# mailgun/gubernator

Hardware: AMD Instinct MI355X
Metric: rate-limit decisions/sec (kernel path, inputs resident in HBM) (higher is better)
Workload: dtype int64

## Files before the change

gubernator_amd/csrc/guber_engine.hip:

```cpp
#include <hip/hip_runtime.h>

#include <algorithm>
#include <atomic>
#include <chrono>
#include <cstdio>
#include <cstdlib>
#include <cstring>
#include <memory>
#include <mutex>
#include <string>
#include <thread>
#include <unordered_map>
#include <vector>

#include "../../include/guber_gpu.h"
#include "guber_host.h"
#include "guber_test_flags.h"
#include "guber_kernels.h"
#include "guber_kernels_lru.h"
#include "guber_item_conv.h"
#include <hipcub/hipcub.hpp>

using namespace guber;

// ... 119 lines not shown
    DevBuf<LruCtl> lru_ctl; PinBuf<LruCtl> lru_hctl;
    DevBuf<unsigned long long> lru_tstamp, lru_tstamp_in, lru_cnt; DevBuf<uint32_t> lru_tslot, lru_tslot_in; DevBuf<uint8_t> lru_sort_tmp;
    DevBuf<unsigned long long> lru_u64; DevBuf<uint32_t> lru_u32; DevBuf<uint8_t> lru_u8;
    bool lru_tail_ok = false;
    uint64_t lru_admits = 0, lru_applied = 0, lru_rebuilds = 0, lru_cuts = 0, lru_passes = 0; uint32_t lru_split_at = 0;
    uint64_t touch = 0;
    static constexpr uint32_t kRb = 32;
    struct RbSlot { uint32_t seq = 0; uint64_t mark = 0; bool armed = false; };
    RbSlot rb[kRb + 1]; int rb_ride = -1;
    uint64_t added_total = 0;
    uint64_t settle_waits = 0;
    uint64_t compactions = 0;
    std::mutex mu;
    bool profiling = false;
    struct Span { int kernel; hipEvent_t a, b; hipStream_t st; };
    std::vector<Span> spans;
    std::vector<hipEvent_t> event_pool;
    double prof_ms[32] = {0}; uint64_t prof_n[32] = {0}, prof_units[32] = {0};
    std::vector<float> group_us;

    hipEvent_t get_event() {
        if (!event_pool.empty()) { hipEvent_t ev = event_pool.back(); event_pool.pop_back(); return ev; }
        hipEvent_t ev = nullptr; (void)hipEventCreate(&ev); return ev;
    }
    void span_begin(int k, uint64_t units = 0, hipStream_t st = nullptr) { if (profiling) { Span s{k, get_event(), get_event(), st ? st : stream}; (void)hipEventRecord(s.a, s.st); spans.push_back(s); prof_units[k] += units; } }
    void span_end() { if (profiling) (void)hipEventRecord(spans.back().b, spans.back().st); }

    mutable struct PendingEval* held = nullptr;
    int set_device() const { if (held) ep_flush_held(this); return hipSetDevice(device) == hipSuccess ? 0 : -1; }
};

enum { KT_FRONT = 0, KT_EVAL2, KT_RESOLVE, KT_HIST, KT_SCATTER0, KT_SCATTER, KT_HEADS, KT_EVAL, KT_FRONT_MULTI, KT_EVAL2_MULTI,
       KT_PART, KT_OWN, KT_EVAL3, KT_PART_MULTI, KT_OWN_MULTI, KT_EVAL3_MULTI, KT_EVALPART_MULTI, KT_FR_COUNT, KT_FR_SCAN, KT_FR_SCATTER, KT_FR_OUT,
       KT_FR_ELECT, KT_FR_MISSING, KT_FR_ASK, KT_FR_OUT_STORE, KT_COUNT };
static_assert(KT_COUNT <= 32, "guber_engine::prof_* hold 32 kernels");
static const char* const kKernelNames[KT_COUNT] = {"k_front", "k_eval2", "k_resolve", "k_hist", "k_scatter(first)",
                                                   "k_scatter", "k_heads", "k_eval", "k_front_multi", "k_eval2_multi",
                                                   "k_part", "k_own", "k_eval3", "k_part_multi", "k_own_multi", "k_eval3_multi", "k_evalpart_multi",
                                                   "k_fr_count", "k_fr_scan", "k_fr_scatter", "k_fr_out",
                                                   "k_fr_elect", "k_fr_missing", "k_fr_ask", "k_fr_out_store"};

static uint64_t take_stamps(guber_engine* e, uint64_t n) {
    const uint64_t b = e->seq_next;
    e->seq_next += n ? n : 1;
    e->touch = b;
    return b;
}
static uint64_t next_pow2(uint64_t v) { uint64_t p = 1; while (p < v) p <<= 1; return p; }

static void quiesce_all(guber_engine* e) { (void)hipStreamSynchronize(e->stream); }

static void note_enqueued(guber_engine* e, uint64_t n) { e->size_upper += n; e->tags_upper += n; e->added_total += n; }
static bool rb_slot_done(const guber_engine* e, uint32_t i) {
    return __atomic_load_n((volatile uint32_t*)&e->h_rb_seq.p[i], __ATOMIC_ACQUIRE) == e->rb[i].seq;
}
static bool rb_any_armed(const guber_engine* e) { for (uint32_t i = 0; i < guber_engine::kRb; ++i) if (e->rb[i].armed) return true; return false; }
static bool rb_any_launched(const guber_engine* e) {
    for (uint32_t i = 0; i < guber_engine::kRb; ++i) if (e->rb[i].armed && (int)i != e->rb_ride) return true;
    return false;
}
static void rb_disarm_all(guber_engine* e) { for (auto& s : e->rb) s.armed = false; e->rb_ride = -1; }
static void rb_fold_slot(guber_engine* e, uint32_t i) {
    DevCounters c = e->h_ctr.p[i];
    const BlockCounters* hb = e->h_bctr.p + (size_t)i * e->n_bctr;
    for (uint32_t b = 0; b < e->n_bctr; ++b) { c.over += hb[b].over; c.hits += hb[b].hits; c.misses += hb[b].misses; c.size += hb[b].size_delta; }
    const uint64_t since = e->added_total - e->rb[i].mark;
    e->last_ctr = c;
    e->tags_upper = c.tags_used + since;
    e->size_upper = (uint64_t)std::max<long long>(c.size, 0) + since;
}
static bool rb_fold_newest(guber_engine* e) {
    int best = -1;
    for (uint32_t i = 0; i < guber_engine::kRb; ++i) {
// ... 244 lines not shown
```

gubernator_amd/csrc/guber_front.h:

```cpp
#pragma once
#include "guber_kernels_wire.h"

constexpr uint32_t FRONT_ONE_PAIR_MAX = 49152;
struct guber_front {
    std::mutex mu;
    int device = 0;
    std::vector<guber_engine*> eng;
    std::vector<hipStream_t> streams;
    std::vector<int> stream_of;
    const guber::WireEnc* enc_hook = nullptr;
    hipStream_t rs = nullptr, rs2 = nullptr, os = nullptr, last_os = nullptr; int n_own_streams = 1; bool out_on_eval = false; uint32_t out_delay = 0, one_pair_max = FRONT_ONE_PAIR_MAX; bool rs_borrowed = false;
    uint32_t cap = 0, depth = 0, max_key = 0;
    uint32_t seq = 0;
    DevBuf<uint16_t> rt_table, rt_exs; DevBuf<uint64_t> rt_exh; RouteRule rule{}; bool have_rule = false;
    struct Slot {
        DevBuf<uint8_t> mem; CohBuf<FrontHost> host;
        FrIn in{};
        uint8_t *o_status = nullptr, *o_err = nullptr; int64_t *o_limit = nullptr, *o_remaining = nullptr, *o_reset = nullptr;
        hipEvent_t ev_in = nullptr, ev_out = nullptr, ev_a = nullptr; bool out_recorded = false;
        std::vector<std::unique_ptr<EvalHook>> hooks;
        CohBuf<uint8_t> h_margs; DevBuf<uint8_t> d_margs;
        uint32_t seq = 0, n = 0;
        int64_t gen = -1;
        bool dispatched = false;
    };
    std::vector<Slot> slots;
    uint64_t generations = 0, forced_flushes = 0, host_waits = 0; double host_wait_ms = 0;
    bool pre_routed = false;
    struct GenSpan { hipEvent_t a, b; };
    std::vector<GenSpan> gen_spans;
    struct StoreSide {
        uint32_t cap = 0, cells = 0;
        DevBuf<unsigned long long> tag; DevBuf<uint32_t> first, cell, tile_cnt, index; DevBuf<uint8_t> ask, engine, flags, oflags; DevBuf<Rec> after, oafter;
        DevBuf<FrStoreCtl> ctl; DevBuf<FrStoreTabs> tabs; FrStoreTabs h_tabs{}; FrStoreCtl h_ctl{};
        std::vector<hipEvent_t> ev;
        bool probed = false, active = false;
        uint32_t n = 0, cut_at = 0; const void *key_bytes = nullptr, *key_off = nullptr; int64_t now_ms = 0;
        uint64_t probes = 0, collisions = 0, cuts = 0, asked = 0, evals = 0;
    } st;
};

static size_t front_col(size_t bytes) { return (bytes + 63) & ~(size_t)63; }
struct FrontGen { guber_batch_t b; uint32_t key_stride = 0; const uint32_t* key_len = nullptr; };

extern "C" void guber_front_destroy(guber_front_t* f) {
    if (!f) return;
    (void)hipSetDevice(f->device);
    for (hipStream_t st : {f->rs, f->rs2, f->os}) if (st) (void)hipStreamSynchronize(st);
    for (auto st : f->streams) (void)hipStreamSynchronize(st);
    for (auto& s : f->slots) {
// ... 32 lines not shown
    f->have_rule = true;
    return 0;
}

extern "C" int guber_front_create(guber_engine_t* const* engines, uint32_t n_engines, const guber_route_rule_t* rule, uint32_t max_n,
                                  uint32_t depth, guber_front_t** out) {
    if (!engines || !out || !n_engines || n_engines > (uint32_t)MULTI_MEM_MAX) return fail(GUBER_E_INVALID_ARG, "1 .. 16 engines per front");
    if (n_engines > 1 && !rule) return fail(GUBER_E_INVALID_ARG, "a front over several engines needs the placement's rule");
    if (max_n == 0 || max_n > FR_MAX_N) return fail(GUBER_E_BATCH_TOO_LARGE, "a generation holds at most 4 194 304 requests");
    if (depth == 0) depth = 4;
    if (depth < 3 || depth > 16) return fail(GUBER_E_INVALID_ARG, "3 .. 16 generations in flight");
    std::unique_ptr<guber_front, void (*)(guber_front*)> f(new guber_front(), [](guber_front* p) { guber_front_destroy(p); });
    for (uint32_t j = 0; j < n_engines; ++j) {
        guber_engine* e = engines[j];
        if (!e) return fail(GUBER_E_INVALID_ARG, "null engine");
        if (e->device != engines[0]->device) return fail(GUBER_E_INVALID_ARG, "the engines of a front live on one device");
        for (uint32_t q = 0; q < j; ++q) if (engines[q] == e) return fail(GUBER_E_INVALID_ARG, "an engine twice in one front");
        f->eng.push_back(e);
        int si = -1;
        for (size_t q = 0; q < f->streams.size(); ++q) if (f->streams[q] == e->stream) si = (int)q;
        if (si < 0) { si = (int)f->streams.size(); f->streams.push_back(e->stream); }
        f->stream_of.push_back(si);
        f->max_key = j == 0 ? e->max_key : std::min(f->max_key, e->max_key);
    }
    f->device = engines[0]->device; f->cap = max_n; f->depth = depth;
    if (hipSetDevice(f->device) != hipSuccess) return fail(GUBER_E_HIP, "hipSetDevice");
    HIPCHK(hipStreamCreateWithFlags(&f->rs, hipStreamNonBlocking));
    f->n_own_streams = 1;
    if (const char* v = guber_lab_env("GUBER_FRONT_STREAMS")) f->n_own_streams = std::max(1, std::min(3, atoi(v)));
    f->out_on_eval = true;
    if (const char* v = guber_lab_env("GUBER_FRONT_OUT_ON_EVAL")) f->out_on_eval = atoi(v) != 0;
    if (const char* v = guber_lab_env("GUBER_FRONT_OUT_DELAY")) f->out_delay = (uint32_t)std::max(0, std::min(2, atoi(v)));
    if (const char* v = guber_lab_env("GUBER_FRONT_ONE_PAIR_MAX")) f->one_pair_max = (uint32_t)strtoul(v, nullptr, 10);
    f->rs2 = f->os = f->rs;
    if (f->n_own_streams >= 2) HIPCHK(hipStreamCreateWithFlags(&f->os, hipStreamNonBlocking));
    if (f->n_own_streams >= 3) HIPCHK(hipStreamCreateWithFlags(&f->rs2, hipStreamNonBlocking));
    if (rule) { const int rc = front_set_rule(f.get(), rule); if (rc) return rc; }
    else f->rule = RouteRule{1, 1, 0, 0, -1, 0, 0, 0, nullptr, nullptr, nullptr};
    const size_t cap = max_n, tiles = (cap + FR_TILE - 1) / FR_TILE;
    f->slots.resize(depth);
    for (auto& s : f->slots) {
        const size_t bytes = 3 * front_col(cap * 4 + 4) + 5 * front_col(cap * 8) + front_col(cap * 4) + 2 * front_col(cap) +
                             3 * front_col(cap * 8) + 2 * front_col(cap) +
                             front_col(cap * FR_KEY_COPY_MAX + 64) +
                             front_col(cap * 2) + 2 * front_col(tiles * MULTI_MEM_MAX * 4) + front_col(sizeof(FrontCtl));
        if (s.mem.ensure(bytes) || s.host.ensure(1)) return GUBER_E_NOMEM;
        if (f->streams.size() == 1 && n_engines > 1 && (s.h_margs.ensure(sizeof(MultiArgsMem)) || s.d_margs.ensure(sizeof(MultiArgsMem)))) return GUBER_E_NOMEM;
        uint8_t* p = s.mem.p;
        FrIn& A = s.in;
        A.d_key_off = (uint32_t*)p; p += front_col(cap * 4 + 4); A.d_key_len = (uint32_t*)p; p += front_col(cap * 4 + 4); A.d_fwd = (uint32_t*)p; p += front_col(cap * 4 + 4);
        A.d_hits = (int64_t*)p; p += front_col(cap * 8); A.d_limit = (int64_t*)p; p += front_col(cap * 8); A.d_duration = (int64_t*)p; p += front_col(cap * 8);
        A.d_burst = (int64_t*)p; p += front_col(cap * 8); A.d_created_at = (int64_t*)p; p += front_col(cap * 8);
        A.d_behavior = (uint32_t*)p; p += front_col(cap * 4); A.d_algorithm = p; p += front_col(cap); A.d_is_owner = p; p += front_col(cap);
        s.o_limit = (int64_t*)p; p += front_col(cap * 8); s.o_remaining = (int64_t*)p; p += front_col(cap * 8); s.o_reset = (int64_t*)p; p += front_col(cap * 8);
        s.o_status = p; p += front_col(cap); s.o_err = p; p += front_col(cap);
        A.d_keys = p; p += front_col(cap * FR_KEY_COPY_MAX + 64);
        A.er = (uint16_t*)p; p += front_col(cap * 2);
        A.tile_cnt = (uint32_t*)p; p += front_col(tiles * MULTI_MEM_MAX * 4); A.tile_base = (uint32_t*)p; p += front_col(tiles * MULTI_MEM_MAX * 4);
        A.ctl = (FrontCtl*)p; p += front_col(sizeof(FrontCtl));
        A.host = s.host.p;
        memset((void*)s.host.p, 0, sizeof(FrontHost));
        HIPCHK(hipMemsetAsync(A.ctl, 0, sizeof(FrontCtl), f->rs));
        HIPCHK(hipMemsetAsync(A.d_keys, 0, front_col(cap * FR_KEY_COPY_MAX + 64), f->rs));
        HIPCHK(hipEventCreateWithFlags(&s.ev_in, hipEventDisableTiming));
        HIPCHK(hipEventCreateWithFlags(&s.ev_out, hipEventDisableTiming));
        for (size_t q = 0; q < f->streams.size(); ++q) {
            s.hooks.emplace_back(new EvalHook());
            HIPCHK(hipEventCreateWithFlags(&s.hooks.back()->ev, hipEventDisableTiming));
            s.hooks.back()->st = f->streams[q];
        }
    }
    HIPCHK(hipStreamSynchronize(f->rs));
    *out = f.release();
    return GUBER_OK;
}

static int front_route_on(guber_front* f, hipStream_t st) {
    std::lock_guard<std::mutex> lk(f->mu);
    if (f->generations || f->pre_routed || f->n_own_streams != 1) return fail(GUBER_E_INVALID_ARG, "guber_front: the routing stream is chosen before the first generation");
    if (hipSetDevice(f->device) != hipSuccess) return fail(GUBER_E_HIP, "hipSetDevice");
    HIPCHK(hipStreamSynchronize(f->rs));
    HIPCHK(hipStreamDestroy(f->rs));
    f->rs = f->rs2 = f->os = st; f->rs_borrowed = true;
    return 0;
}

extern "C" int guber_front_set_rule(guber_front_t* f, const guber_route_rule_t* rule) {
    if (!f || !rule) return fail(GUBER_E_INVALID_ARG, "null argument");
    std::lock_guard<std::mutex> lk(f->mu);
    if (hipSetDevice(f->device) != hipSuccess) return fail(GUBER_E_HIP, "hipSetDevice");
    return front_set_rule(f, rule);
}

static int front_route(guber_front* f, guber_front::Slot& s, const FrontGen* fg, int64_t gen) {
    const guber_batch_t* b = &fg->b;
    hipStream_t rs = (gen & 1) ? f->rs2 : f->rs;
    if (s.out_recorded) { HIPCHK(hipStreamWaitEvent(rs, s.ev_out, 0)); s.out_recorded = false; }
    s.gen = gen; s.n = b->n; s.dispatched = false;
    s.seq = ++f->seq ? f->seq : ++f->seq;
    for (auto& h : s.hooks) { h->outstanding.store(1); h->recorded.store(false); }
    if (b->n == 0) return 0;
    FrIn& A = s.in;
    A.n = b->n; A.n_engines = (uint32_t)f->eng.size(); A.max_key = f->max_key; A.seq = s.seq;
    A.key_bytes = b->key_bytes; A.key_off = b->key_off; A.key_stride = fg->key_stride; A.key_len = fg->key_len; A.hits = b->hits; A.limit = b->limit; A.duration = b->duration;
    A.burst = b->burst; A.created_at = b->created_at; A.behavior = b->behavior; A.algorithm = b->algorithm; A.is_owner = b->is_owner;
    A.R = f->rule;
    const uint32_t tiles = (b->n + FR_TILE - 1u) / FR_TILE;
    guber_engine* e0 = f->eng[0];
    std::unique_lock<std::mutex> pl(e0->mu, std::defer_lock);
    if (e0->profiling || s.ev_a) pl.lock();
    if (s.ev_a) e0->event_pool.push_back(s.ev_a);
    s.ev_a = nullptr;
    if (e0->profiling) { s.ev_a = e0->get_event(); (void)hipEventRecord(s.ev_a, rs); }
    e0->span_begin(KT_FR_COUNT, b->n, rs);
    hipLaunchKernelGGL(k_fr_count, dim3(tiles), dim3(FR_TILE), 0, rs, A);
    e0->span_end();
    e0->span_begin(KT_FR_SCAN, b->n, rs);
    hipLaunchKernelGGL(k_fr_scan, dim3(MULTI_MEM_MAX / 4), dim3(FR_SCAN_T), 0, rs, A, tiles, (tiles + FR_SCAN_T - 1) / FR_SCAN_T);
    e0->span_end();
    e0->span_begin(KT_FR_SCATTER, b->n, rs);
    hipLaunchKernelGGL(k_fr_scatter, dim3(tiles), dim3(256), 0, rs, A);
    e0->span_end();
    if (hipGetLastError() != hipSuccess) return fail(GUBER_E_HIP, "kernel launch");
    HIPCHK(hipEventRecord(s.ev_in, rs));
    return 0;
}

static int front_out(guber_front* f, guber_front::Slot& s, guber_result_t* r) {
    if (s.n == 0) return 0;
    hipStream_t os = f->out_on_eval ? f->streams[(size_t)s.gen % f->streams.size()] : f->os;
    f->last_os = os;
    for (auto& h : s.hooks) if (h->st != os) HIPCHK(hipStreamWaitEvent(os, h->ev, 0));
    FrOut O{};
    O.n = s.n; O.er = s.in.er; O.tile_cnt = s.in.tile_cnt; O.tile_base = s.in.tile_base; O.ctl = s.in.ctl;
    O.d_status = s.o_status; O.d_err = s.o_err; O.d_limit = s.o_limit; O.d_remaining = s.o_remaining; O.d_reset_time = s.o_reset;
    O.status = r->status; O.err = r->err; O.limit = r->limit; O.remaining = r->remaining; O.reset_time = r->reset_time;
    guber_engine* e0 = f->eng[0];
    std::unique_lock<std::mutex> pl(e0->mu, std::defer_lock);
    if (e0->profiling) pl.lock();
    e0->span_begin(f->st.active ? KT_FR_OUT_STORE : KT_FR_OUT, s.n, os);
    if (f->st.active) {
        FrOutStore S{O, f->st.flags.p, f->st.after.p, f->st.oflags.p, f->st.oafter.p};
        hipLaunchKernelGGL(k_fr_out_store, dim3((s.n + FR_TILE - 1u) / FR_TILE), dim3(256), 0, os, S);
    } else if (f->enc_hook) {
        guber::WireEnc E = *f->enc_hook;
        E.fwd = s.in.d_fwd; E.d_status = O.d_status; E.d_err = O.d_err; E.d_limit = O.d_limit; E.d_remaining = O.d_remaining; E.d_reset = O.d_reset_time;
        hipLaunchKernelGGL(guber::k_wire_enc, dim3(E.nrpc), dim3(guber::WE_T), 0, os, E);
    } else
    hipLaunchKernelGGL(k_fr_out, dim3((s.n + FR_TILE - 1u) / FR_TILE), dim3(256), 0, os, O);
    e0->span_end();
    if (s.ev_a) { hipEvent_t evb = e0->get_event(); (void)hipEventRecord(evb, os); f->gen_spans.push_back({s.ev_a, evb}); s.ev_a = nullptr; }
    if (hipGetLastError() != hipSuccess) return fail(GUBER_E_HIP, "kernel launch");
    if (os != f->rs) { HIPCHK(hipEventRecord(s.ev_out, os)); s.out_recorded = true; }
    return 0;
}

static bool front_evals_launched(const guber_front::Slot& s) {
    for (auto& h : s.hooks) if (!h->recorded.load(std::memory_order_acquire)) return false;
    return true;
}

static int front_eval(guber_front* f, const FrontGen* gens, guber_result_t* results, uint32_t count, uint32_t* done, hipEvent_t after = nullptr);
extern "C" int guber_front_eval_dev(guber_front_t* f, const guber_batch_t* gens, guber_result_t* results, uint32_t count, uint32_t* done) {
    if (done) *done = 0;
    if (!f || (count && (!gens || !results))) return fail(GUBER_E_INVALID_ARG, "null argument");
    std::vector<FrontGen> g(count);
    for (uint32_t k = 0; k < count; ++k) {
        const int rc = check_batch_args(&gens[k], &results[k]);
        if (rc) return rc;
        g[k].b = gens[k];
    }
    return front_eval(f, g.data(), results, count, done);
}
static int front_eval_locked(guber_front* f, const FrontGen* gens, guber_result_t* results, uint32_t count, uint32_t* done, hipEvent_t after);
static int front_eval(guber_front* f, const FrontGen* gens, guber_result_t* results, uint32_t count, uint32_t* done, hipEvent_t after) {
    if (done) *done = 0;
    for (uint32_t k = 0; k < count; ++k) {
        if (gens[k].b.n > f->cap) return fail(GUBER_E_BATCH_TOO_LARGE, "generation larger than the front was created for");
        if (gens[k].b.greg_expire || gens[k].b.greg_duration) return fail(GUBER_E_INVALID_ARG, "a front takes its calendar intervals from the device");
// ... 8 lines not shown
    if (f->st.probed && !f->st.active) { f->st.probed = false; f->pre_routed = false; }
    const uint32_t ne = (uint32_t)f->eng.size(), D = f->depth, ahead = D - 2;
    PendSet pendset;
    bool any_ep = false;
    for (auto* e : f->eng) any_ep = any_ep || e->fuse_ep;
    PendSet* const ps = any_ep ? &pendset : nullptr;
    struct Dispatching { bool on; Dispatching(bool o) : on(o) { if (on) ++tl_ep_dispatcher; } ~Dispatching() { if (on) --tl_ep_dispatcher; } } dispatching(any_ep);
    uint32_t next_route = 0, next_out = 0, enq = 0;
    int rc = 0;
    uint64_t fp[4] = {0, 0, 0, 0};
    struct FpSpan { uint64_t* a; uint64_t t0; explicit FpSpan(uint64_t* x) : a(x), t0(dp_now()) {} ~FpSpan() { if (g_dprof) *a += dp_now() - t0; } };
    const uint64_t g0 = f->generations;
    auto slot_of = [&](uint32_t k) -> guber_front::Slot& { return f->slots[(g0 + k) % D]; };
    auto drain_outs = [&](uint32_t upto, bool force) -> int {
        while (next_out < upto) {
            guber_front::Slot& s = slot_of(next_out);
            if (!s.dispatched) break;
            if (s.n && !front_evals_launched(s)) {
                if (!force) break;
                f->forced_flushes++;
                const int r2 = pendset.flush_all();
                if (r2) return r2;
                if (!front_evals_launched(s)) return fail(GUBER_E_HIP, "guber_front: an evaluation was not launched");
            }
            const int r3 = front_out(f, s, &results[next_out]);
            if (r3) return r3;
            ++next_out;
            if (done) *done = next_out;
        }
        return 0;
    };
    std::vector<std::vector<GroupItem>> fifo(ne);
    std::vector<EvalHook*> hook_of(ne, nullptr);
    for (uint32_t k = 0; k < count && !rc; ++k) {
        while (next_route < count && next_route <= k + ahead && !rc) {
            if (next_route >= D) { rc = drain_outs(next_route - D + 1, true); if (rc) break; }
            if (next_route == 0 && f->pre_routed) f->pre_routed = false;
            else { FpSpan sp(&fp[0]); rc = front_route(f, slot_of(next_route), &gens[next_route], (int64_t)f->generations + next_route); }
            ++next_route;
        }
        if (rc) break;
        guber_front::Slot& s = slot_of(k);
        const guber_batch_t* b = &gens[k].b;
        if (s.n) {
            auto reported = [&]() {
                for (int q = 0; q <= MULTI_MEM_MAX; ++q)
                    if ((uint32_t)(__atomic_load_n((volatile unsigned long long*)&s.host.p->w[q], __ATOMIC_ACQUIRE) >> 32) != s.seq) return false;
                return true;
            };
            if (!reported()) {
                FpSpan sp(&fp[1]);
                const auto t0 = std::chrono::steady_clock::now();
                f->host_waits++;
                uint32_t spins = 0;
                while (!reported()) {
                    if (++spins > 2000) {
                        std::this_thread::yield();
                        if ((spins & 0x3ffu) == 0 && hipStreamQuery((s.gen & 1) ? f->rs2 : f->rs) != hipErrorNotReady && !reported()) {
                            rc = fail(GUBER_E_HIP, "guber_front: the routing of a generation did not report"); break;
                        }
                    }
                }
                f->host_wait_ms += std::chrono::duration<double, std::milli>(std::chrono::steady_clock::now() - t0).count();
                if (rc) break;
            }
            uint32_t counts[MULTI_MEM_MAX];
            for (int q = 0; q < MULTI_MEM_MAX; ++q) counts[q] = (uint32_t)s.host.p->w[q];
            const bool packed = !((uint32_t)s.host.p->w[MULTI_MEM_MAX] >> 8 & 1u);
            for (auto st : f->streams) { if (hipStreamWaitEvent(st, s.ev_in, 0) != hipSuccess) { rc = fail(GUBER_E_HIP, "hipStreamWaitEvent"); break; } }
            if (rc) break;
            uint32_t base = 0, total = 0;
            for (uint32_t j = 0; j < ne; ++j) {
                fifo[j].clear();
// ... 6 lines not shown
                uint32_t piece = np > 1 ? ((nj + np - 1) / np + 255u) & ~255u : cap_e;
                if (piece > cap_e) piece = cap_e;
                for (uint32_t pos = 0; pos < nj; pos += piece) {
                    const uint32_t len = std::min(piece, nj - pos), d0 = base + pos;
                    const FrIn& A = s.in;
                    BatchView B{len, 0, packed ? A.d_keys : b->key_bytes, A.d_key_off + d0, A.d_hits + d0, A.d_limit + d0, A.d_duration + d0,
                                b->burst ? A.d_burst + d0 : nullptr, b->created_at ? A.d_created_at + d0 : nullptr,
                                A.d_algorithm + d0, A.d_behavior + d0, b->is_owner ? A.d_is_owner + d0 : nullptr, nullptr, nullptr, b->now_ms,
                                0, packed ? nullptr : A.d_key_len + d0};
                    fifo[j].push_back(GroupItem{B, ResultView{s.o_status + d0, s.o_limit + d0, s.o_remaining + d0, s.o_reset + d0, s.o_err + d0},
                                                f->st.active ? f->st.flags.p + d0 : nullptr, f->st.active ? f->st.after.p + d0 : nullptr});
                }
                base += nj;
            }
            if (total != s.n) { rc = fail(GUBER_E_HIP, "guber_front: the shares do not add up to the generation"); break; }
            bool one_pair = f->streams.size() == 1 && ne > 1 && s.h_margs.p && s.n <= f->one_pair_max;
            guber_engine* og[MULTI_MEM_MAX]; GroupItem oi[MULTI_MEM_MAX]; int on = 0;
            for (uint32_t j = 0; j < ne && one_pair; ++j) {
                if (fifo[j].empty()) continue;
                one_pair = fifo[j].size() == 1 && can_fuse(f->eng[j], fifo[j][0].B.n);
                og[on] = f->eng[j]; oi[on] = fifo[j][0]; ++on;
            }
            if (one_pair && on > 1) {
                FpSpan sp(&fp[2]);
                rc = pendset.flush_all();
                int r1 = rc ? rc : launch_group_mem(og, oi, on, &enq, (MultiArgsMem*)s.h_margs.p, (MultiArgsMem*)s.d_margs.p);
                if (r1 == 1) r1 = dispatch_rounds(f->eng.data(), ne, fifo, ps, &enq, hook_of.data());
                rc = r1;
            } else { FpSpan sp(&fp[2]); rc = dispatch_rounds(f->eng.data(), ne, fifo, ps, &enq, hook_of.data()); }
        }
        s.dispatched = true;
        for (auto& h : s.hooks) h->launched();
        if (rc) break;
        { FpSpan sp(&fp[3]); rc = drain_outs(k + 1 > f->out_delay ? k + 1 - f->out_delay : 0, false); }
    }
    {
        for (uint32_t k = 0; k < next_route; ++k) {
            guber_front::Slot& s = slot_of(k);
            if (k >= next_out && !s.dispatched) { s.dispatched = true; s.n = 0; for (auto& h : s.hooks) h->launched(); }
        }
        const int rcf = pendset.flush_all();
        if (!rc) rc = rcf;
        const int rco = drain_outs(next_route, true);
        if (!rc) rc = rco;
    }
    f->generations += next_out;
    if (after && !rc && hipEventRecord(after, f->last_os ? f->last_os : f->rs) != hipSuccess) rc = fail(GUBER_E_HIP, "hipEventRecord");
    if (g_dprof && next_out) {
        fprintf(stderr, "[front] %u generations; per generation: routing enqueue %.2f us, waiting for the shares' sizes %.2f, dispatch %.2f, answers %.2f\n", next_out,
                fp[0] / 1e3 / next_out, fp[1] / 1e3 / next_out, fp[2] / 1e3 / next_out, fp[3] / 1e3 / next_out);
        if (tl_dp[6]) fprintf(stderr, "[front dispatch] %llu batches in %llu groups; per batch: wait-for-progress %.2f us, locks %.2f, preludes+plans %.2f, argument blocks %.2f, launches %.2f\n",
                (unsigned long long)tl_dp[6], (unsigned long long)tl_dp[5], tl_dp[0] / 1e3 / tl_dp[6], tl_dp[1] / 1e3 / tl_dp[6], tl_dp[2] / 1e3 / tl_dp[6],
                tl_dp[3] / 1e3 / tl_dp[6], tl_dp[4] / 1e3 / tl_dp[6]);
        for (auto& v : tl_dp) v = 0;
    }
    return rc;
}

static int front_route_ahead(guber_front* f, const FrontGen* g) {
    if (g->b.n > f->cap) return fail(GUBER_E_BATCH_TOO_LARGE, "generation larger than the front was created for");
    if (g->key_stride & 7u) return fail(GUBER_E_INVALID_ARG, "key rows are a multiple of 8 bytes apart");
    std::lock_guard<std::mutex> lk(f->mu);
    if (f->st.probed) { f->st.probed = false; f->pre_routed = false; }
    if (f->pre_routed) return fail(GUBER_E_INVALID_ARG, "guber_front: a generation is routed ahead already");
    if (hipSetDevice(f->device) != hipSuccess) return fail(GUBER_E_HIP, "hipSetDevice");
    const int rc = front_route(f, f->slots[f->generations % f->depth], g, (int64_t)f->generations);
    if (!rc) f->pre_routed = true;
    return rc;
}
// ... 243 lines not shown
```

gubernator_amd/csrc/guber_kernels_front.h:

```cpp
#pragma once

namespace guber {

constexpr uint32_t FR_PER = 4;
constexpr uint32_t FR_TILE = 256 * FR_PER;
constexpr uint32_t FR_RANK_BITS = 10;
static_assert((1u << FR_RANK_BITS) >= FR_TILE && (MULTI_MEM_MAX << FR_RANK_BITS) <= 65536, "engine and rank share sixteen bits");
constexpr uint32_t FR_SCAN_T = 1024;
constexpr uint32_t FR_SCAN_PER = 4;
constexpr uint32_t FR_MAX_N = FR_SCAN_T * FR_SCAN_PER * FR_TILE;
constexpr uint32_t FR_KEY_COPY_MAX = 32;

struct FrontCtl {
    uint32_t tot[MULTI_MEM_MAX];
    uint32_t ragged_seq;
    uint32_t pad_[15];
};
struct FrontHost { unsigned long long w[MULTI_MEM_MAX + 1]; unsigned long long pad_[15]; };
static_assert(sizeof(FrontHost) == 256, "four lines of pinned memory per slot");

struct FrIn {
    uint32_t n, n_engines, max_key, seq;
    const uint8_t* key_bytes; const uint32_t* key_off;
    uint32_t key_stride; const uint32_t* key_len;
// ... 78 lines not shown
        const uint32_t ragged = __hip_atomic_load(&A.ctl->ragged_seq, __ATOMIC_RELAXED, __HIP_MEMORY_SCOPE_AGENT) == A.seq ? 1u : 0u;
        const uint32_t len0 = fr_len0(A);
        __hip_atomic_store(&A.host->w[MULTI_MEM_MAX], (unsigned long long)A.seq << 32 | ragged << 8 | (len0 < 255u ? len0 : 255u), __ATOMIC_RELAXED, __HIP_MEMORY_SCOPE_SYSTEM);
    }
}

struct FrTile { uint32_t lbase[MULTI_MEM_MAX + 1], dofs[MULTI_MEM_MAX]; };
__device__ __forceinline__ void fr_tile_bases(FrTile& T, const FrontCtl* ctl, const uint32_t* tile_cnt, const uint32_t* tile_base, uint32_t tile) {
    const uint32_t e = threadIdx.x;
    if (e < MULTI_MEM_MAX) {
        const uint32_t* cnt = tile_cnt + (size_t)tile * MULTI_MEM_MAX;
        uint32_t s = 0, l = 0;
        for (uint32_t k = 0; k < e; ++k) { s += ctl->tot[k]; l += cnt[k]; }
        T.lbase[e] = l; T.dofs[e] = s + tile_base[(size_t)tile * MULTI_MEM_MAX + e] - l;
        if (e == MULTI_MEM_MAX - 1) T.lbase[MULTI_MEM_MAX] = l + cnt[e];
    }
    __syncthreads();
}
__device__ __forceinline__ uint32_t fr_engine_of(const FrTile& T, uint32_t j) {
    uint32_t e = 0;
#pragma unroll
    for (uint32_t q = 1; q < MULTI_MEM_MAX; ++q) e += T.lbase[q] <= j ? 1u : 0u;
    return e;
}
__device__ __forceinline__ void fr_sorted_places(const FrTile& T, uint32_t n, uint32_t (&dd)[FR_PER]) {
    const uint32_t cnt = T.lbase[MULTI_MEM_MAX] < FR_TILE ? T.lbase[MULTI_MEM_MAX] : FR_TILE;
#pragma unroll
    for (int k = 0; k < FR_PER; ++k) {
        const uint32_t j = threadIdx.x + k * 256u, d = T.dofs[fr_engine_of(T, j)] + j;
        dd[k] = j < cnt && d < n ? d : 0xffffffffu;
    }
}

__global__ __launch_bounds__(256) void k_fr_scatter(FrIn A) {
    __shared__ FrTile T;
    __shared__ uint64_t stg[2][FR_TILE];
    const uint32_t tile = blockIdx.x, tid = threadIdx.x, i0 = tile * FR_TILE + tid;
    fr_tile_bases(T, A.ctl, A.tile_cnt, A.tile_base, tile);
    const bool packed = A.ctl->ragged_seq != A.seq;
    const uint32_t len0 = fr_len0(A), ko0 = A.key_stride ? 0u : A.key_off[0], kstep = A.key_stride ? A.key_stride : len0;
    uint32_t p[FR_PER], o0[FR_PER], klen[FR_PER]; uint64_t hits[FR_PER], limit[FR_PER], duration[FR_PER], misc[FR_PER], kw[FR_PER];
    auto word_at = [](uint32_t w, uint32_t len) { return 8u * w + 8u <= len || len < 8u ? 8u * w : len - 8u; };
#pragma unroll
    for (int k = 0; k < FR_PER; ++k) {
        const uint32_t i = i0 + k * 256u;
        p[k] = 0xffffffffu; o0[k] = klen[k] = 0; hits[k] = limit[k] = duration[k] = misc[k] = kw[k] = 0;
        if (i >= A.n) continue;
        const uint32_t er = A.er[i];
        if (packed) { o0[k] = ko0 + i * kstep; klen[k] = len0; kw[k] = ld_key_word(A.key_bytes + o0[k]); }
        else { o0[k] = fr_key_off(A, i); klen[k] = fr_key_len(A, i, o0[k]); }
        hits[k] = (uint64_t)A.hits[i]; limit[k] = (uint64_t)A.limit[i]; duration[k] = (uint64_t)A.duration[i];
        misc[k] = (A.behavior ? A.behavior[i] : 0u) | (uint64_t)(A.algorithm ? A.algorithm[i] : (uint8_t)0) << 32 | (uint64_t)(A.is_owner ? A.is_owner[i] : (uint8_t)0) << 40;
        const uint32_t e = er >> FR_RANK_BITS;
        p[k] = T.lbase[e] + (er & ((1u << FR_RANK_BITS) - 1u));
        const uint32_t d = T.dofs[e] + p[k];
        A.d_fwd[i] = d < A.n ? d : 0u;
    }
    uint32_t dd[FR_PER];
    fr_sorted_places(T, A.n, dd);
    uint32_t turn = 0;
    auto through = [&](const uint64_t (&v)[FR_PER], uint64_t (&o)[FR_PER]) {
        uint64_t* buf = stg[turn++ & 1u];
#pragma unroll
        for (int k = 0; k < FR_PER; ++k) if (p[k] < FR_TILE) buf[p[k]] = v[k];
        __syncthreads();
#pragma unroll
        for (int k = 0; k < FR_PER; ++k) o[k] = dd[k] != 0xffffffffu ? buf[threadIdx.x + k * 256u] : 0ull;
    };
    auto column = [&](const uint64_t (&v)[FR_PER], int64_t* dst) {
        uint64_t o[FR_PER];
        through(v, o);
#pragma unroll
        for (int k = 0; k < FR_PER; ++k) if (dd[k] != 0xffffffffu) dst[dd[k]] = (int64_t)o[k];
    };
    uint64_t opt[FR_PER] = {0, 0, 0, 0}, o[FR_PER];
    auto request = [&](const int64_t* src) {
#pragma unroll
        for (int k = 0; k < FR_PER; ++k) if (p[k] != 0xffffffffu) opt[k] = (uint64_t)src[i0 + k * 256u];
    };
    column(hits, A.d_hits);
    column(limit, A.d_limit);
    if (A.burst) request(A.burst);
    column(duration, A.d_duration);
    if (A.burst) column(opt, A.d_burst);
    if (A.created_at) request(A.created_at);
    through(misc, o);
#pragma unroll
    for (int k = 0; k < FR_PER; ++k) {
        if (dd[k] == 0xffffffffu) continue;
// ... 4 lines not shown
    if (packed) {
        const uint32_t nw = (len0 + 7u) >> 3;
        for (uint32_t w = 0; w < nw; ++w) {
            uint64_t next[FR_PER] = {0, 0, 0, 0};
            if (w + 1 < nw) {
#pragma unroll
                for (int k = 0; k < FR_PER; ++k) if (p[k] != 0xffffffffu) next[k] = ld_key_word(A.key_bytes + o0[k] + word_at(w + 1, len0));
            }
            through(kw, o);
#pragma unroll
            for (int k = 0; k < FR_PER; ++k) {
                kw[k] = next[k];
                if (dd[k] == 0xffffffffu) continue;
                uint8_t* dst = A.d_keys + (size_t)dd[k] * len0;
                if (len0 >= 8) __builtin_memcpy(dst + word_at(w, len0), &o[k], 8);
                else for (uint32_t q = 0; q < len0; ++q) dst[q] = (uint8_t)(o[k] >> (8 * q));
            }
        }
#pragma unroll
        for (int k = 0; k < FR_PER; ++k) {
            if (dd[k] == 0xffffffffu) continue;
            A.d_key_off[dd[k]] = dd[k] * len0;
            if (dd[k] == A.n - 1) A.d_key_off[A.n] = A.n * len0;
        }
    } else {
        uint64_t ol[FR_PER];
#pragma unroll
        for (int k = 0; k < FR_PER; ++k) ol[k] = o0[k] | (uint64_t)klen[k] << 32;
        through(ol, o);
#pragma unroll
        for (int k = 0; k < FR_PER; ++k) if (dd[k] != 0xffffffffu) { A.d_key_off[dd[k]] = (uint32_t)o[k]; A.d_key_len[dd[k]] = (uint32_t)(o[k] >> 32); }
    }
}

struct FrOut {
    uint32_t n; const uint16_t* er; const uint32_t *tile_cnt, *tile_base; const FrontCtl* ctl;
    const uint8_t *d_status, *d_err; const int64_t *d_limit, *d_remaining, *d_reset_time;
    uint8_t *status, *err; int64_t *limit, *remaining, *reset_time;
};
__global__ __launch_bounds__(256) void k_fr_out(FrOut A) {
    __shared__ FrTile T;
    __shared__ uint64_t stg[2][FR_TILE];
    __shared__ uint16_t sse[FR_TILE];
    const uint32_t tile = blockIdx.x, tid = threadIdx.x, i0 = tile * FR_TILE + tid;
    fr_tile_bases(T, A.ctl, A.tile_cnt, A.tile_base, tile);
    uint32_t dd[FR_PER], p[FR_PER]; uint16_t se[FR_PER]; int64_t l[FR_PER], r[FR_PER], t[FR_PER];
    fr_sorted_places(T, A.n, dd);
#pragma unroll
    for (int k = 0; k < FR_PER; ++k) {
        p[k] = 0xffffffffu;
        if (i0 + k * 256u < A.n) { const uint32_t er = A.er[i0 + k * 256u]; p[k] = T.lbase[er >> FR_RANK_BITS] + (er & ((1u << FR_RANK_BITS) - 1u)); }
        if (p[k] >= FR_TILE) p[k] = 0xffffffffu;
        se[k] = 0; l[k] = r[k] = t[k] = 0;
        if (dd[k] == 0xffffffffu) continue;
        se[k] = (uint16_t)(A.d_status[dd[k]] | A.d_err[dd[k]] << 8); l[k] = A.d_limit[dd[k]]; r[k] = A.d_remaining[dd[k]]; t[k] = A.d_reset_time[dd[k]];
    }
#pragma unroll
    for (int k = 0; k < FR_PER; ++k) { stg[0][tid + k * 256u] = (uint64_t)l[k]; sse[tid + k * 256u] = se[k]; }
    __syncthreads();
#pragma unroll
    for (int k = 0; k < FR_PER; ++k) {
        if (p[k] == 0xffffffffu) continue;
        const uint32_t i = i0 + k * 256u; const uint16_t v = sse[p[k]];
        A.limit[i] = (int64_t)stg[0][p[k]]; A.status[i] = (uint8_t)v; A.err[i] = (uint8_t)(v >> 8);
    }
#pragma unroll
    for (int k = 0; k < FR_PER; ++k) stg[1][tid + k * 256u] = (uint64_t)r[k];
    __syncthreads();
#pragma unroll
    for (int k = 0; k < FR_PER; ++k) if (p[k] != 0xffffffffu) A.remaining[i0 + k * 256u] = (int64_t)stg[1][p[k]];
#pragma unroll
    for (int k = 0; k < FR_PER; ++k) stg[0][tid + k * 256u] = (uint64_t)t[k];
    __syncthreads();
#pragma unroll
    for (int k = 0; k < FR_PER; ++k) if (p[k] != 0xffffffffu) A.reset_time[i0 + k * 256u] = (int64_t)stg[0][p[k]];
}

}
```

gubernator_amd/csrc/guber_wire_pool.h:

```cpp
#pragma once
#include <linux/futex.h>
#include <sys/syscall.h>
#include <unistd.h>
#include <sched.h>
#include <sys/resource.h>
#include <climits>

#ifndef GUBER_WPL_WALK_MAX
#define GUBER_WPL_WALK_MAX 8192
#endif
namespace {
constexpr uint64_t WPL_CLOSED = 1ull << 63;
constexpr uint32_t WPL_MAX_RPCS = 4095, WPL_MAX_ITEMS = (1u << 20) - 1, WPL_MAX_B16 = (1u << 20) - 1, WPL_NONE = 15, WPL_MAX_STAGES = 12;
inline uint32_t wpl_gen(uint64_t w) { return (uint32_t)(w >> 52) & 0x7ffu; }
inline uint32_t wpl_rpcs(uint64_t w) { return (uint32_t)(w >> 40) & 0xfffu; }
inline uint32_t wpl_items(uint64_t w) { return (uint32_t)(w >> 20) & 0xfffffu; }
inline uint32_t wpl_b16(uint64_t w) { return (uint32_t)w & 0xfffffu; }
inline uint64_t wpl_word(uint32_t gen, uint32_t rpcs, uint32_t items, uint32_t b16) {
    return ((uint64_t)(gen & 0x7ffu) << 52) | ((uint64_t)rpcs << 40) | ((uint64_t)items << 20) | b16;
}
inline void wpl_futex_wait(std::atomic<uint32_t>* w, uint32_t seen, int64_t timeout_us) {
    struct timespec ts; ts.tv_sec = timeout_us / 1000000; ts.tv_nsec = (timeout_us % 1000000) * 1000;
    syscall(SYS_futex, (uint32_t*)w, FUTEX_WAIT_PRIVATE, seen, timeout_us < 0 ? nullptr : &ts, nullptr, 0);
}
// ... 318 lines not shown
extern "C" int guber_wire_pool_create(guber_engine_t* const* engines, uint32_t n_engines, const guber_route_rule_t* rule, const guber_wire_pool_config_t* cfg,
                                      guber_wire_pool_t** out) {
    if (!engines || !n_engines || !out) return fail(GUBER_E_INVALID_ARG, "null argument");
    *out = nullptr;
    guber_wire_pool_config_t c{};
    if (cfg) c = *cfg;
    if (!c.stages) c.stages = 12;
    if (!c.max_items) c.max_items = 49152;
    if (!c.max_payload_bytes) c.max_payload_bytes = 8u << 20;
    if (!c.max_rpcs) c.max_rpcs = 1024;
    if (!c.batch_wait_us) c.batch_wait_us = 500;
    if (!c.max_per_rpc) c.max_per_rpc = 1000;
    if (!c.spin_us) c.spin_us = 150;
    if (!c.decodes_queued) c.decodes_queued = 2;
    if (c.stages < 2 || c.stages > WPL_MAX_STAGES || c.max_items > WPL_MAX_ITEMS || c.max_rpcs > WPL_MAX_RPCS || c.max_payload_bytes / 16 > WPL_MAX_B16 || c.max_payload_bytes < 64)
        return fail(GUBER_E_INVALID_ARG, "guber_wire_pool: 2 .. 12 stages of at most 1 048 575 items, 4 095 RPCs and 16 MiB of payload bytes");
    std::unique_ptr<guber_wire_pool, void (*)(guber_wire_pool*)> p(new guber_wire_pool(), [](guber_wire_pool* q) { guber_wire_pool_destroy(q); });
    for (uint32_t j = 0; j < n_engines; ++j) { if (!engines[j]) return fail(GUBER_E_INVALID_ARG, "null engine"); p->eng.push_back(engines[j]); }
    p->device = engines[0]->device;
    p->n_stages = c.stages; p->max_items = c.max_items; p->max_b16 = c.max_payload_bytes / 16; p->max_rpcs = c.max_rpcs; p->wait_us = c.batch_wait_us;
    p->max_per_rpc = c.max_per_rpc == 0xffffffffu ? 0 : c.max_per_rpc; p->spin_us = c.spin_us; p->decodes = c.decodes_queued;
    p->cpus = wpl_usable_cpus();
    if (rule && n_engines > 1) {
        if (rule->n_shards == 0 || rule->per == 0 || !rule->table || (rule->ex_cells & (rule->ex_cells - 1)) || (rule->ex_n && (!rule->ex_hash || !rule->ex_shard || rule->ex_n >= rule->ex_cells)))
            return fail(GUBER_E_INVALID_ARG, "malformed route rule");
        guber_wire_pool::HostRule& H = p->hrule;
        H.n_shards = rule->n_shards; H.per = rule->per; H.ex_cells = rule->ex_cells; H.ex_n = rule->ex_n; H.global_engine = rule->global_engine;
        H.step = rule->step; H.inv_step = rule->inv_step; H.inv_sub = rule->inv_sub;
        H.table.assign(rule->table, rule->table + (size_t)rule->n_shards * rule->per);
        if (rule->ex_n) { H.ex_hash.assign(rule->ex_hash, rule->ex_hash + rule->ex_cells); H.ex_shard.assign(rule->ex_shard, rule->ex_shard + rule->ex_cells); }
    }
    p->item_cap = std::min<uint32_t>(std::min<uint32_t>(c.max_items, 4096u), p->max_per_rpc ? p->max_per_rpc : 4096u);
    {
        const int rc = guber_front_create(engines, n_engines, rule, c.max_items, 4, &p->front);
        if (rc) return rc;
    }
    if (hipSetDevice(p->device) != hipSuccess) return fail(GUBER_E_HIP, "hipSetDevice");
#ifdef GUBER_LAB
    {
        if (const char* dv = guber_lab_env("GUBER_WIRE_DIRECT")) p->direct_max = (uint32_t)atoi(dv);
        const char* he = guber_lab_env("GUBER_WIRE_HOST_ENCODE");
        p->host_encode = he && atoi(he) != 0;
        const char* v = guber_lab_env("GUBER_WIRE_ROUTE_ON_ENGINES");
        bool one = true;
        for (uint32_t j = 1; j < n_engines; ++j) one = one && engines[j]->stream == engines[0]->stream;
        if (v && atoi(v) != 0 && one) { const int rc = front_route_on(p->front, engines[0]->stream); if (rc) return rc; }
    }
#endif
    HIPCHK(hipStreamCreateWithFlags(&p->ws[0], hipStreamNonBlocking));
    if (c.decodes_queued > 1) HIPCHK(hipStreamCreateWithFlags(&p->ws[1], hipStreamNonBlocking));
    p->stages.reset(new guber_wire_pool::Stage[c.stages]);
    const size_t M = c.max_items, R = c.max_rpcs;
    for (uint32_t k = 0; k < c.stages; ++k) {
        guber_wire_pool::Stage& s = p->stages[k];
        int rc = guber_wire_dev_create(engines[k % n_engines], c.max_items, c.max_payload_bytes, c.max_rpcs, &s.dec);
        if (rc) return rc;
        rc = guber_wire_dev_set_stream(s.dec, p->ws[1] ? p->ws[k & 1] : p->ws[0]);
        if (rc) return rc;
        size_t cap = 0;
        rc = guber_wire_dev_buffer(s.dec, &s.buf, &cap);
        if (rc) return rc;
        const size_t col8 = (M + 63) & ~(size_t)63;
        if (s.meta.ensure(2 * R) || s.owner.ensure(R) || s.res.ensure(2 * col8 + 3 * 8 * M + 64) || s.enc.ensure(guber::wire_enc_bytes(c.max_items, c.max_rpcs)) || s.enc_len.ensure(R))
            return GUBER_E_NOMEM;
        s.status.resize(R); s.first.resize(R); s.count.resize(R);
        uint8_t* q = s.res.p;
        s.r = guber_result_t{};
// ... 239 lines not shown
```

Baseline: 5.244 billion.

## Split front routing and fuse next scatter with previous output kernel

Splits front routing into a count/scan phase and a deferred scatter phase. When the GUBER_FRONT_OUT_ROLE knob is set, the next generation's scatter is fused with the previous generation's output gather into one kernel launch, cutting launch count and stream serialization. Separately, the forward-index write is skipped unless a wire encoder was declared, which removes a global store per item on the default path. The pairing adds scheduling complexity around out-drain ordering and event waits.

```diff
diff --git a/gubernator_amd/csrc/guber_engine.hip b/gubernator_amd/csrc/guber_engine.hip
--- a/gubernator_amd/csrc/guber_engine.hip
+++ b/gubernator_amd/csrc/guber_engine.hip
@@ -175,13 +175,13 @@
 
 enum { KT_FRONT = 0, KT_EVAL2, KT_RESOLVE, KT_HIST, KT_SCATTER0, KT_SCATTER, KT_HEADS, KT_EVAL, KT_FRONT_MULTI, KT_EVAL2_MULTI,
        KT_PART, KT_OWN, KT_EVAL3, KT_PART_MULTI, KT_OWN_MULTI, KT_EVAL3_MULTI, KT_EVALPART_MULTI, KT_FR_COUNT, KT_FR_SCAN, KT_FR_SCATTER, KT_FR_OUT,
-       KT_FR_ELECT, KT_FR_MISSING, KT_FR_ASK, KT_FR_OUT_STORE, KT_COUNT };
+       KT_FR_ELECT, KT_FR_MISSING, KT_FR_ASK, KT_FR_OUT_STORE, KT_FR_SCATTER_OUT, KT_COUNT };
 static_assert(KT_COUNT <= 32, "guber_engine::prof_* hold 32 kernels");
 static const char* const kKernelNames[KT_COUNT] = {"k_front", "k_eval2", "k_resolve", "k_hist", "k_scatter(first)",
                                                    "k_scatter", "k_heads", "k_eval", "k_front_multi", "k_eval2_multi",
                                                    "k_part", "k_own", "k_eval3", "k_part_multi", "k_own_multi", "k_eval3_multi", "k_evalpart_multi",
                                                    "k_fr_count", "k_fr_scan", "k_fr_scatter", "k_fr_out",
-                                                   "k_fr_elect", "k_fr_missing", "k_fr_ask", "k_fr_out_store"};
+                                                   "k_fr_elect", "k_fr_missing", "k_fr_ask", "k_fr_out_store", "k_fr_scatter_out"};
 
 static uint64_t take_stamps(guber_engine* e, uint64_t n) {
     const uint64_t b = e->seq_next;
diff --git a/gubernator_amd/csrc/guber_front.h b/gubernator_amd/csrc/guber_front.h
--- a/gubernator_amd/csrc/guber_front.h
+++ b/gubernator_amd/csrc/guber_front.h
@@ -10,12 +10,14 @@
     std::vector<int> stream_of;
     const guber::WireEnc* enc_hook = nullptr;
     hipStream_t rs = nullptr, rs2 = nullptr, os = nullptr, last_os = nullptr; int n_own_streams = 1; bool out_on_eval = false; uint32_t out_delay = 0, one_pair_max = FRONT_ONE_PAIR_MAX; bool rs_borrowed = false;
+    bool out_role = false, has_encoder = false;
     uint32_t cap = 0, depth = 0, max_key = 0;
     uint32_t seq = 0;
     DevBuf<uint16_t> rt_table, rt_exs; DevBuf<uint64_t> rt_exh; RouteRule rule{}; bool have_rule = false;
     struct Slot {
         DevBuf<uint8_t> mem; CohBuf<FrontHost> host;
         FrIn in{};
+        uint32_t* fwd = nullptr;
         uint8_t *o_status = nullptr, *o_err = nullptr; int64_t *o_limit = nullptr, *o_remaining = nullptr, *o_reset = nullptr;
         hipEvent_t ev_in = nullptr, ev_out = nullptr, ev_a = nullptr; bool out_recorded = false;
         std::vector<std::unique_ptr<EvalHook>> hooks;
@@ -114,6 +116,7 @@
     if (const char* v = guber_lab_env("GUBER_FRONT_OUT_ON_EVAL")) f->out_on_eval = atoi(v) != 0;
     if (const char* v = guber_lab_env("GUBER_FRONT_OUT_DELAY")) f->out_delay = (uint32_t)std::max(0, std::min(2, atoi(v)));
     if (const char* v = guber_lab_env("GUBER_FRONT_ONE_PAIR_MAX")) f->one_pair_max = (uint32_t)strtoul(v, nullptr, 10);
+    if (const char* v = guber_lab_env("GUBER_FRONT_OUT_ROLE")) f->out_role = atoi(v) != 0;
     f->rs2 = f->os = f->rs;
     if (f->n_own_streams >= 2) HIPCHK(hipStreamCreateWithFlags(&f->os, hipStreamNonBlocking));
     if (f->n_own_streams >= 3) HIPCHK(hipStreamCreateWithFlags(&f->rs2, hipStreamNonBlocking));
@@ -130,7 +133,7 @@
         if (f->streams.size() == 1 && n_engines > 1 && (s.h_margs.ensure(sizeof(MultiArgsMem)) || s.d_margs.ensure(sizeof(MultiArgsMem)))) return GUBER_E_NOMEM;
         uint8_t* p = s.mem.p;
         FrIn& A = s.in;
-        A.d_key_off = (uint32_t*)p; p += front_col(cap * 4 + 4); A.d_key_len = (uint32_t*)p; p += front_col(cap * 4 + 4); A.d_fwd = (uint32_t*)p; p += front_col(cap * 4 + 4);
+        A.d_key_off = (uint32_t*)p; p += front_col(cap * 4 + 4); A.d_key_len = (uint32_t*)p; p += front_col(cap * 4 + 4); s.fwd = (uint32_t*)p; p += front_col(cap * 4 + 4);
         A.d_hits = (int64_t*)p; p += front_col(cap * 8); A.d_limit = (int64_t*)p; p += front_col(cap * 8); A.d_duration = (int64_t*)p; p += front_col(cap * 8);
         A.d_burst = (int64_t*)p; p += front_col(cap * 8); A.d_created_at = (int64_t*)p; p += front_col(cap * 8);
         A.d_behavior = (uint32_t*)p; p += front_col(cap * 4); A.d_algorithm = p; p += front_col(cap); A.d_is_owner = p; p += front_col(cap);
@@ -174,7 +177,15 @@
     return front_set_rule(f, rule);
 }
 
-static int front_route(guber_front* f, guber_front::Slot& s, const FrontGen* fg, int64_t gen) {
+#define GUBER_FRONT_DECLARES_ENCODER 1
+static int front_declare_encoder(guber_front* f) {
+    std::lock_guard<std::mutex> lk(f->mu);
+    if (f->generations || f->pre_routed) return fail(GUBER_E_INVALID_ARG, "guber_front: an encoder is declared before the first generation");
+    f->has_encoder = true;
+    return 0;
+}
+
+static int front_route_count(guber_front* f, guber_front::Slot& s, const FrontGen* fg, int64_t gen) {
     const guber_batch_t* b = &fg->b;
     hipStream_t rs = (gen & 1) ? f->rs2 : f->rs;
     if (s.out_recorded) { HIPCHK(hipStreamWaitEvent(rs, s.ev_out, 0)); s.out_recorded = false; }
@@ -186,6 +197,7 @@
     A.n = b->n; A.n_engines = (uint32_t)f->eng.size(); A.max_key = f->max_key; A.seq = s.seq;
     A.key_bytes = b->key_bytes; A.key_off = b->key_off; A.key_stride = fg->key_stride; A.key_len = fg->key_len; A.hits = b->hits; A.limit = b->limit; A.duration = b->duration;
     A.burst = b->burst; A.created_at = b->created_at; A.behavior = b->behavior; A.algorithm = b->algorithm; A.is_owner = b->is_owner;
+    A.d_fwd = f->has_encoder ? s.fwd : nullptr;
     A.R = f->rule;
     const uint32_t tiles = (b->n + FR_TILE - 1u) / FR_TILE;
     guber_engine* e0 = f->eng[0];
@@ -200,12 +212,42 @@
     e0->span_begin(KT_FR_SCAN, b->n, rs);
     hipLaunchKernelGGL(k_fr_scan, dim3(MULTI_MEM_MAX / 4), dim3(FR_SCAN_T), 0, rs, A, tiles, (tiles + FR_SCAN_T - 1) / FR_SCAN_T);
     e0->span_end();
-    e0->span_begin(KT_FR_SCATTER, b->n, rs);
-    hipLaunchKernelGGL(k_fr_scatter, dim3(tiles), dim3(256), 0, rs, A);
+    if (hipGetLastError() != hipSuccess) return fail(GUBER_E_HIP, "kernel launch");
+    return 0;
+}
+static void front_out_args(FrOut& O, const guber_front::Slot& s, const guber_result_t* r) {
+    O.n = s.n; O.er = s.in.er; O.tile_cnt = s.in.tile_cnt; O.tile_base = s.in.tile_base; O.ctl = s.in.ctl;
+    O.d_status = s.o_status; O.d_err = s.o_err; O.d_limit = s.o_limit; O.d_remaining = s.o_remaining; O.d_reset_time = s.o_reset;
+    O.status = r->status; O.err = r->err; O.limit = r->limit; O.remaining = r->remaining; O.reset_time = r->reset_time;
+}
+static int front_route_scatter(guber_front* f, guber_front::Slot& s, guber_front::Slot* o = nullptr, const guber_result_t* r = nullptr) {
+    if (s.n == 0) return 0;
+    hipStream_t rs = (s.gen & 1) ? f->rs2 : f->rs;
+    const uint32_t tiles = (s.n + FR_TILE - 1u) / FR_TILE;
+    FrOut O{};
+    if (o) {
+        for (auto& h : o->hooks) if (h->st != rs) HIPCHK(hipStreamWaitEvent(rs, h->ev, 0));
+        front_out_args(O, *o, r);
+    }
+    guber_engine* e0 = f->eng[0];
+    std::unique_lock<std::mutex> pl(e0->mu, std::defer_lock);
+    if (e0->profiling) pl.lock();
+    e0->span_begin(o ? KT_FR_SCATTER_OUT : KT_FR_SCATTER, (uint64_t)s.n + (o ? o->n : 0u), rs);
+    if (o) {
+        const uint32_t tiles_o = (o->n + FR_TILE - 1u) / FR_TILE;
+        hipLaunchKernelGGL(k_fr_scatter_out, dim3(tiles + tiles_o), dim3(256), 0, rs, s.in, O, tiles, tiles_o);
+    } else
+    hipLaunchKernelGGL(k_fr_scatter, dim3(tiles), dim3(256), 0, rs, s.in);
     e0->span_end();
+    if (o && o->ev_a) { hipEvent_t evb = e0->get_event(); (void)hipEventRecord(evb, rs); f->gen_spans.push_back({o->ev_a, evb}); o->ev_a = nullptr; }
     if (hipGetLastError() != hipSuccess) return fail(GUBER_E_HIP, "kernel launch");
     HIPCHK(hipEventRecord(s.ev_in, rs));
+    if (o) f->last_os = rs;
     return 0;
+}
+static int front_route(guber_front* f, guber_front::Slot& s, const FrontGen* fg, int64_t gen) {
+    const int rc = front_route_count(f, s, fg, gen);
+    return rc ? rc : front_route_scatter(f, s);
 }
 
 static int front_out(guber_front* f, guber_front::Slot& s, guber_result_t* r) {
@@ -213,10 +255,9 @@
     hipStream_t os = f->out_on_eval ? f->streams[(size_t)s.gen % f->streams.size()] : f->os;
     f->last_os = os;
     for (auto& h : s.hooks) if (h->st != os) HIPCHK(hipStreamWaitEvent(os, h->ev, 0));
+    if (f->enc_hook && !f->has_encoder) return fail(GUBER_E_INVALID_ARG, "guber_front: an encoder hook on a front whose owner declared none");
     FrOut O{};
-    O.n = s.n; O.er = s.in.er; O.tile_cnt = s.in.tile_cnt; O.tile_base = s.in.tile_base; O.ctl = s.in.ctl;
-    O.d_status = s.o_status; O.d_err = s.o_err; O.d_limit = s.o_limit; O.d_remaining = s.o_remaining; O.d_reset_time = s.o_reset;
-    O.status = r->status; O.err = r->err; O.limit = r->limit; O.remaining = r->remaining; O.reset_time = r->reset_time;
+    front_out_args(O, s, r);
     guber_engine* e0 = f->eng[0];
     std::unique_lock<std::mutex> pl(e0->mu, std::defer_lock);
     if (e0->profiling) pl.lock();
@@ -226,7 +267,7 @@
         hipLaunchKernelGGL(k_fr_out_store, dim3((s.n + FR_TILE - 1u) / FR_TILE), dim3(256), 0, os, S);
     } else if (f->enc_hook) {
         guber::WireEnc E = *f->enc_hook;
-        E.fwd = s.in.d_fwd; E.d_status = O.d_status; E.d_err = O.d_err; E.d_limit = O.d_limit; E.d_remaining = O.d_remaining; E.d_reset = O.d_reset_time;
+        E.fwd = s.fwd; E.d_status = O.d_status; E.d_err = O.d_err; E.d_limit = O.d_limit; E.d_remaining = O.d_remaining; E.d_reset = O.d_reset_time;
         hipLaunchKernelGGL(guber::k_wire_enc, dim3(E.nrpc), dim3(guber::WE_T), 0, os, E);
     } else
     hipLaunchKernelGGL(k_fr_out, dim3((s.n + FR_TILE - 1u) / FR_TILE), dim3(256), 0, os, O);
@@ -301,13 +342,29 @@
     };
     std::vector<std::vector<GroupItem>> fifo(ne);
     std::vector<EvalHook*> hook_of(ne, nullptr);
+    const bool pairing = f->out_role && !f->enc_hook && !f->st.active && f->n_own_streams == 1 && f->out_delay == 0 && count >= 2 * D;
+    int64_t pend = -1;
+    auto scatter_pend = [&](guber_front::Slot* o, const guber_result_t* r) -> int {
+        if (pend < 0) return 0;
+        FpSpan sp(&fp[0]);
+        const int r1 = front_route_scatter(f, slot_of((uint32_t)pend), o, r);
+        pend = -1;
+        return r1;
+    };
     for (uint32_t k = 0; k < count && !rc; ++k) {
         while (next_route < count && next_route <= k + ahead && !rc) {
+            rc = scatter_pend(nullptr, nullptr);
+            if (rc) break;
             if (next_route >= D) { rc = drain_outs(next_route - D + 1, true); if (rc) break; }
             if (next_route == 0 && f->pre_routed) f->pre_routed = false;
-            else { FpSpan sp(&fp[0]); rc = front_route(f, slot_of(next_route), &gens[next_route], (int64_t)f->generations + next_route); }
+            else {
+                FpSpan sp(&fp[0]);
+                rc = front_route_count(f, slot_of(next_route), &gens[next_route], (int64_t)f->generations + next_route);
+                if (!rc) pend = next_route;
+            }
             ++next_route;
         }
+        if (!rc && pend >= 0 && (!pairing || pend <= (int64_t)k)) rc = scatter_pend(nullptr, nullptr);
         if (rc) break;
         guber_front::Slot& s = slot_of(k);
         const guber_batch_t* b = &gens[k].b;
@@ -380,9 +437,23 @@
         s.dispatched = true;
         for (auto& h : s.hooks) h->launched();
         if (rc) break;
-        { FpSpan sp(&fp[3]); rc = drain_outs(k + 1 > f->out_delay ? k + 1 - f->out_delay : 0, false); }
+        if (pend >= 0) {
+            guber_front::Slot* o = nullptr;
+            if (k >= 1 && next_out == k - 1 && slot_of((uint32_t)pend).n) {
+                guber_front::Slot& so = slot_of(k - 1);
+                if (so.dispatched && so.n && front_evals_launched(so)) o = &so;
+            }
+            rc = scatter_pend(o, o ? &results[k - 1] : nullptr);
+            if (rc) break;
+            if (o) { ++next_out; if (done) *done = next_out; }
+        }
+        const uint32_t rn = k + 1 + ahead;
+        const bool ride = pairing && s.n && rn < count && gens[rn].b.n;
+        { FpSpan sp(&fp[3]); rc = drain_outs(ride ? k : k + 1 > f->out_delay ? k + 1 - f->out_delay : 0, false); }
     }
     {
+        const int rcs = scatter_pend(nullptr, nullptr);
+        if (!rc) rc = rcs;
         for (uint32_t k = 0; k < next_route; ++k) {
             guber_front::Slot& s = slot_of(k);
             if (k >= next_out && !s.dispatched) { s.dispatched = true; s.n = 0; for (auto& h : s.hooks) h->launched(); }
diff --git a/gubernator_amd/csrc/guber_kernels_front.h b/gubernator_amd/csrc/guber_kernels_front.h
--- a/gubernator_amd/csrc/guber_kernels_front.h
+++ b/gubernator_amd/csrc/guber_kernels_front.h
@@ -134,10 +134,8 @@
     }
 }
 
-__global__ __launch_bounds__(256) void k_fr_scatter(FrIn A) {
-    __shared__ FrTile T;
-    __shared__ uint64_t stg[2][FR_TILE];
-    const uint32_t tile = blockIdx.x, tid = threadIdx.x, i0 = tile * FR_TILE + tid;
+__device__ __forceinline__ void fr_scatter_tile(const FrIn& A, const uint32_t tile, FrTile& T, uint64_t (&stg)[2][FR_TILE]) {
+    const uint32_t tid = threadIdx.x, i0 = tile * FR_TILE + tid;
     fr_tile_bases(T, A.ctl, A.tile_cnt, A.tile_base, tile);
     const bool packed = A.ctl->ragged_seq != A.seq;
     const uint32_t len0 = fr_len0(A), ko0 = A.key_stride ? 0u : A.key_off[0], kstep = A.key_stride ? A.key_stride : len0;
@@ -156,7 +154,7 @@
         const uint32_t e = er >> FR_RANK_BITS;
         p[k] = T.lbase[e] + (er & ((1u << FR_RANK_BITS) - 1u));
         const uint32_t d = T.dofs[e] + p[k];
-        A.d_fwd[i] = d < A.n ? d : 0u;
+        if (A.d_fwd) A.d_fwd[i] = d < A.n ? d : 0u;
     }
     uint32_t dd[FR_PER];
     fr_sorted_places(T, A.n, dd);
@@ -227,17 +225,19 @@
         for (int k = 0; k < FR_PER; ++k) if (dd[k] != 0xffffffffu) { A.d_key_off[dd[k]] = (uint32_t)o[k]; A.d_key_len[dd[k]] = (uint32_t)(o[k] >> 32); }
     }
 }
+__global__ __launch_bounds__(256) void k_fr_scatter(FrIn A) {
+    __shared__ FrTile T;
+    __shared__ uint64_t stg[2][FR_TILE];
+    fr_scatter_tile(A, blockIdx.x, T, stg);
+}
 
 struct FrOut {
     uint32_t n; const uint16_t* er; const uint32_t *tile_cnt, *tile_base; const FrontCtl* ctl;
     const uint8_t *d_status, *d_err; const int64_t *d_limit, *d_remaining, *d_reset_time;
     uint8_t *status, *err; int64_t *limit, *remaining, *reset_time;
 };
-__global__ __launch_bounds__(256) void k_fr_out(FrOut A) {
-    __shared__ FrTile T;
-    __shared__ uint64_t stg[2][FR_TILE];
-    __shared__ uint16_t sse[FR_TILE];
-    const uint32_t tile = blockIdx.x, tid = threadIdx.x, i0 = tile * FR_TILE + tid;
+__device__ __forceinline__ void fr_out_tile(const FrOut& A, const uint32_t tile, FrTile& T, uint64_t (&stg)[2][FR_TILE], uint16_t (&sse)[FR_TILE]) {
+    const uint32_t tid = threadIdx.x, i0 = tile * FR_TILE + tid;
     fr_tile_bases(T, A.ctl, A.tile_cnt, A.tile_base, tile);
     uint32_t dd[FR_PER], p[FR_PER]; uint16_t se[FR_PER]; int64_t l[FR_PER], r[FR_PER], t[FR_PER];
     fr_sorted_places(T, A.n, dd);
@@ -270,5 +270,23 @@
 #pragma unroll
     for (int k = 0; k < FR_PER; ++k) if (p[k] != 0xffffffffu) A.reset_time[i0 + k * 256u] = (int64_t)stg[0][p[k]];
 }
-
-}
+__global__ __launch_bounds__(256) void k_fr_out(FrOut A) {
+    __shared__ FrTile T;
+    __shared__ uint64_t stg[2][FR_TILE];
+    __shared__ uint16_t sse[FR_TILE];
+    fr_out_tile(A, blockIdx.x, T, stg, sse);
+}
+
+struct FrLds { FrTile T; uint64_t stg[2][FR_TILE]; uint16_t sse[FR_TILE]; };
+static_assert(sizeof(FrLds) == 18568, "FrTile + two buffers of 8 KB + the 16-bit column");
+static_assert(sizeof(FrIn) + sizeof(FrOut) + 8 <= 4096, "kernel arguments are limited to 4 KB");
+__global__ __launch_bounds__(256) void k_fr_scatter_out(FrIn A, FrOut O, uint32_t tiles_s, uint32_t tiles_o) {
+    __shared__ FrLds L;
+    const uint32_t b = blockIdx.x, both = tiles_s < tiles_o ? tiles_s : tiles_o;
+    const bool out = b < 2u * both ? (b & 1u) != 0u : tiles_o > tiles_s;
+    const uint32_t tile = b < 2u * both ? b >> 1 : b - both;
+    if (out) fr_out_tile(O, tile, L.T, L.stg, L.sse);
+    else fr_scatter_tile(A, tile, L.T, L.stg);
+}
+
+}
diff --git a/gubernator_amd/csrc/guber_wire_pool.h b/gubernator_amd/csrc/guber_wire_pool.h
--- a/gubernator_amd/csrc/guber_wire_pool.h
+++ b/gubernator_amd/csrc/guber_wire_pool.h
@@ -374,7 +374,10 @@
     }
     p->item_cap = std::min<uint32_t>(std::min<uint32_t>(c.max_items, 4096u), p->max_per_rpc ? p->max_per_rpc : 4096u);
     {
-        const int rc = guber_front_create(engines, n_engines, rule, c.max_items, 4, &p->front);
+        int rc = guber_front_create(engines, n_engines, rule, c.max_items, 4, &p->front);
+#ifdef GUBER_FRONT_DECLARES_ENCODER
+        if (!rc) rc = front_declare_encoder(p->front);
+#endif
         if (rc) return rc;
     }
     if (hipSetDevice(p->device) != hipSuccess) return fail(GUBER_E_HIP, "hipSetDevice");
```

New measurement: 5.186 billion. 0.989x the previous value.
